# zhaoruiyang98/eftpipe

Hardware: AMD Instinct MI355X
Metric: theory P_l(k) evaluations/sec (single tracer, Nk=512, l=0,2,4) (higher is better)
Workload: dtype f64

## Files before the change

eftpipe_amd/csrc/eftb_kernels.hpp:

```cpp
#pragma once
#include <hip/hip_runtime.h>
#include <stdint.h>
#include <stdlib.h>

namespace eftb {

constexpr int NS = 80;
constexpr int NPOW = 257;
constexpr int NHALF = 128;
constexpr int NCH = 129;

constexpr int NROW = 24;

typedef double v4d __attribute__((ext_vector_type(4)));
typedef double v2d __attribute__((ext_vector_type(2)));

__device__ __forceinline__ void xcd_decode(int ntile, int& tile, int& group) {
    const int flat = blockIdx.x, ng = gridDim.x / ntile;
    if ((ng & 7) == 0) {
        const int slot = flat >> 3;
        tile = slot % ntile;
        group = (flat & 7) + 8 * (slot / ntile);
    } else {
        tile = flat % ntile;
        group = flat / ntile;
    }
}

template <bool LO>
__device__ __forceinline__ void prep_rows_body(int Nkin, int ntail, int nxtail, int KP1, int KP2, int KP3, int Bmax,
                                                        const double* __restrict__ Pin, const double* __restrict__ lnkin,
                                                        const double* __restrict__ lnxtail, const double* __restrict__ lnxxtail,
                                                        const double* __restrict__ wq2, double* __restrict__ A1, double* __restrict__ A2,
                                                        double* __restrict__ A2T, double* __restrict__ A3, int* __restrict__ status,
                                                        int ntail_lo, int nxtail_lo) {
    extern __shared__ double sm[];
    double* pin = sm;
    const int w = blockIdx.x, tid = threadIdx.x;
    bool bad = false;
    for (int j = tid; j < Nkin; j += blockDim.x) {
        const double v = Pin[(size_t)w * Nkin + j];
        pin[j] = v;
        bad = bad || !(fabs(v) <= 1.79769313486231570815e308) || (j >= Nkin - 2 && !(v > 0.0));
        if (LO) bad = bad || (j < 2 && !(v > 0.0));
    }
    if (bad && status) atomicMax(status, w + 1);
    __syncthreads();
    const double dln = lnkin[Nkin - 1] - lnkin[Nkin - 2];
    const double dlo = LO ? lnkin[1] - lnkin[0] : 0.0;
    if (A1) {
        const double slope = (log(pin[Nkin - 1]) - log(pin[Nkin - 2])) / dln;
        const double amp = pin[Nkin - 1] * exp(-slope * lnkin[Nkin - 1]);
        double slo = 0.0, alo = 0.0;
        if (LO && ntail_lo) {
            slo = (log(pin[1]) - log(pin[0])) / dlo;
            alo = pin[0] * exp(-slo * lnkin[0]);
        }
        const int nhi = ntail - (LO ? ntail_lo : 0);
        for (int j = tid; j < KP1; j += blockDim.x) A1[(size_t)w * KP1 + j] = j < Nkin ? pin[j] : 0.0;
        for (int j = tid; j < KP2; j += blockDim.x) {
            double v = j < Nkin ? pin[j] : (j < Nkin + ntail ? amp * exp(slope * lnxtail[j - Nkin]) : 0.0);
            if (LO && j >= Nkin + nhi && j < Nkin + ntail) v = alo * exp(slo * lnxtail[j - Nkin]);
            A2[(size_t)w * KP2 + j] = v;
            A2T[(size_t)j * Bmax + w] = v;
        }
    }
    if (A3) {
        const double q1 = pin[Nkin - 1] * wq2[1], q0 = pin[Nkin - 2] * wq2[0];
        const double slope = (log(q1) - log(q0)) / dln;
        const double amp = q1 * exp(-slope * lnkin[Nkin - 1]);
        double slo = 0.0, alo = 0.0;
        if (LO && nxtail_lo) {
            const double p0 = pin[0] * wq2[2], p1 = pin[1] * wq2[3];
            slo = (log(p1) - log(p0)) / dlo;
            alo = p0 * exp(-slo * lnkin[0]);
        }
        const int nhi = nxtail - (LO ? nxtail_lo : 0);
        for (int j = tid; j < KP3; j += blockDim.x) {
            double v = j < Nkin ? pin[j] : (j < Nkin + nxtail ? amp * exp(slope * lnxxtail[j - Nkin]) : 0.0);
            if (LO && j >= Nkin + nhi && j < Nkin + nxtail) v = alo * exp(slo * lnxxtail[j - Nkin]);
            A3[(size_t)w * KP3 + j] = v;
        }
    }
}

#define PREP_ROWS_PARAMS int Nkin, int ntail, int nxtail, int KP1, int KP2, int KP3, int Bmax, const double* __restrict__ Pin, \
    const double* __restrict__ lnkin, const double* __restrict__ lnxtail, const double* __restrict__ lnxxtail, const double* __restrict__ wq2, \
    double* __restrict__ A1, double* __restrict__ A2, double* __restrict__ A2T, double* __restrict__ A3, int* __restrict__ status
#define PREP_ROWS_ARGS Nkin, ntail, nxtail, KP1, KP2, KP3, Bmax, Pin, lnkin, lnxtail, lnxxtail, wq2, A1, A2, A2T, A3, status

__global__ __launch_bounds__(256) void prep_rows_kernel(PREP_ROWS_PARAMS) {
    prep_rows_body<false>(PREP_ROWS_ARGS, 0, 0);
}

__global__ __launch_bounds__(256) void prep_rows_lo_kernel(PREP_ROWS_PARAMS, int ntail_lo, int nxtail_lo) {
    prep_rows_body<true>(PREP_ROWS_ARGS, ntail_lo, nxtail_lo);
}

__device__ __forceinline__ void qf_body(int w, int nq, const double* __restrict__ fgrow, const double* __restrict__ Qpoly, double* __restrict__ Q) {
    const int tid = threadIdx.x;
    const double f = fgrow[w];
    for (int idx = tid; idx < 2 * nq; idx += blockDim.x) {
        const int a = idx / nq, rest = idx % nq;
        const double* c = Qpoly + ((size_t)(1 - a) * nq + rest) * 15;
        double cv[15];
#pragma unroll
        for (int p = 0; p < 15; ++p) cv[p] = c[p];
        const double f2 = f * f;
        double ev = cv[14], od = cv[13];
#pragma unroll
        for (int p = 12; p >= 0; p -= 2) {
            ev = fma(ev, f2, cv[p]);
            if (p >= 1) od = fma(od, f2, cv[p - 1]);
        }
        Q[(size_t)w * 2 * nq + idx] = fma(od, f, ev);
    }
}

__global__ __launch_bounds__(256) void prep_rows_qf_kernel(int B, PREP_ROWS_PARAMS, int nq, const double* __restrict__ fgrow,
                                                           const double* __restrict__ Qpoly, double* __restrict__ Q) {
    if ((int)blockIdx.x >= B) {
        qf_body(blockIdx.x - B, nq, fgrow, Qpoly, Q);
        return;
    }
    prep_rows_body<false>(PREP_ROWS_ARGS, 0, 0);
}

__global__ __launch_bounds__(256) void prep_rows_qf_lo_kernel(int B, PREP_ROWS_PARAMS, int nq, const double* __restrict__ fgrow,
                                                              const double* __restrict__ Qpoly, double* __restrict__ Q, int ntail_lo, int nxtail_lo) {
    if ((int)blockIdx.x >= B) {
        qf_body(blockIdx.x - B, nq, fgrow, Qpoly, Q);
        return;
    }
    prep_rows_body<true>(PREP_ROWS_ARGS, ntail_lo, nxtail_lo);
}
#undef PREP_ROWS_PARAMS
#undef PREP_ROWS_ARGS

constexpr int AD_T = NHALF + 2;
constexpr int AD_CH = 1;
constexpr int KSYN = 528;
constexpr int KLIN = 288;
constexpr int SYN_KPAD = 48;
constexpr int SYN_KC = 24;
static_assert(SYN_KPAD % SYN_KC == 0 && (32 * SYN_KC) % 256 == 0, "chunk must divide the padding and fill the staging threads");
constexpr int BAS22 = 8, BASC = 32;

__device__ __forceinline__ double readlane_f64(double v, int lane) {
    return __hiloint2double(__builtin_amdgcn_readlane(__double2hiint(v), lane), __builtin_amdgcn_readlane(__double2loint(v), lane));
}

template <int NC, int NW>
__global__ __launch_bounds__(64 * NW) void antidiag_kernel(int B, int Bmax, const double* __restrict__ coefT,
                                                           const double2* __restrict__ AD, double2* __restrict__ S) {
    constexpr int PB = 3, WPP = 2 * NC;
    static_assert(PB * WPP <= 64, "one wave-load must hold a block's weights");
    __shared__ double red[NW - 1][2 * NC][64];
    const int grp = blockIdx.y, jp = (grp & 1) ? NPOW - 1 - (int)blockIdx.x : (int)blockIdx.x;
    const int lane = threadIdx.x & 63, wave = threadIdx.x >> 6, w = grp * 64 + lane;
    const int wl = w < B ? w : B - 1;
    const int cnt = ((2 * NHALF + jp) >> 1) - jp + 1;
    const int per = (cnt + NW - 1) / NW, t0 = wave * per, t1 = min(cnt, t0 + per);
    const double* cr = coefT + wl;
    const double* ci = coefT + (size_t)NCH * Bmax + wl;
    double ar[NC], ai[NC];
#pragma unroll
    for (int q = 0; q < NC; ++q) ar[q] = ai[q] = 0.0;
    if (t0 < t1) {
        const double* adw = reinterpret_cast<const double*>(AD + ((size_t)jp * AD_T + t0) * NC);
        const int nw = (t1 - t0) * WPP;
        auto wload = [&](int blk) { return adw[min(blk * PB * WPP + lane, nw - 1)]; };
        double xr[PB], xi[PB], yr[PB], yi[PB];
        auto coef = [&](int t, int p) {
            const int n = jp + t, qn = n <= NHALF ? n : 2 * NHALF - n;
            xr[p] = cr[(size_t)qn * Bmax];
            xi[p] = ci[(size_t)qn * Bmax];
            yr[p] = cr[(size_t)t * Bmax];
            yi[p] = ci[(size_t)t * Bmax];
        };
        double wc = wload(0);
#pragma unroll
        for (int p = 0; p < PB; ++p) coef(min(t0 + p, t1 - 1), p);
        const int nblk = (t1 - t0 + PB - 1) / PB;
        for (int blk = 0; blk < nblk; ++blk) {
            const double wn = wload(blk + 1);
#pragma unroll
            for (int p = 0; p < PB; ++p) {
                const int t = t0 + blk * PB + p;
                const double on = t < t1 ? 1.0 : 0.0;
                const double xim = jp + t <= NHALF ? xi[p] : -xi[p], yim = -yi[p];
                const double pr = (xr[p] * yr[p] - xim * yim) * on, pi = (xr[p] * yim + xim * yr[p]) * on;
                __builtin_amdgcn_sched_barrier(0);
                coef(min(t + PB, t1 - 1), p);
                __builtin_amdgcn_sched_barrier(0);
#pragma unroll
                for (int q = 0; q < NC; ++q) {
                    const double mx = readlane_f64(wc, p * WPP + 2 * q), my = readlane_f64(wc, p * WPP + 2 * q + 1);
                    ar[q] = fma(mx, pr, fma(-my, pi, ar[q]));
                    ai[q] = fma(mx, pi, fma(my, pr, ai[q]));
                }
                __builtin_amdgcn_sched_barrier(0);
            }
            wc = wn;
        }
    }
    if (wave > 0) {
#pragma unroll
        for (int q = 0; q < NC; ++q) {
            red[wave - 1][2 * q][lane] = ar[q];
            red[wave - 1][2 * q + 1][lane] = ai[q];
        }
    }
    __syncthreads();
    if (wave == 0 && w < B) {
#pragma unroll
        for (int q = 0; q < NC; ++q) {
#pragma unroll
            for (int v = 0; v < NW - 1; ++v) {
                ar[q] += red[v][2 * q][lane];
                ai[q] += red[v][2 * q + 1][lane];
            }
            S[((size_t)w * NC + q) * NPOW + jp] = make_double2(ar[q], ai[q]);
        }
    }
}

template <int NC, int NW>
__global__ __launch_bounds__(64 * NW) void antidiag_nh_kernel(int B, int Bmax, const double* __restrict__ coefT,
                                                              const double2* __restrict__ AD, double2* __restrict__ S, int nh) {
    constexpr int PB = 3, WPP = 2 * NC;
    static_assert(PB * WPP <= 64, "one wave-load must hold a block's weights");
    __shared__ double red[NW - 1][2 * NC][64];
    const int npow = 2 * nh + 1, nch = nh + 1, adt = nh + 2;
    const int grp = blockIdx.y, jp = (grp & 1) ? npow - 1 - (int)blockIdx.x : (int)blockIdx.x;
    const int lane = threadIdx.x & 63, wave = threadIdx.x >> 6, w = grp * 64 + lane;
    const int wl = w < B ? w : B - 1;
    const int cnt = ((2 * nh + jp) >> 1) - jp + 1;
    const int per = (cnt + NW - 1) / NW, t0 = wave * per, t1 = min(cnt, t0 + per);
    const double* cr = coefT + wl;
    const double* ci = coefT + (size_t)nch * Bmax + wl;
    double ar[NC], ai[NC];
#pragma unroll
    for (int q = 0; q < NC; ++q) ar[q] = ai[q] = 0.0;
    if (t0 < t1) {
        const double* adw = reinterpret_cast<const double*>(AD + ((size_t)jp * adt + t0) * NC);
        const int nw = (t1 - t0) * WPP;
        auto wload = [&](int blk) { return adw[min(blk * PB * WPP + lane, nw - 1)]; };
        double xr[PB], xi[PB], yr[PB], yi[PB];
        auto coef = [&](int t, int p) {
            const int n = jp + t, qn = n <= nh ? n : 2 * nh - n;
            xr[p] = cr[(size_t)qn * Bmax];
            xi[p] = ci[(size_t)qn * Bmax];
            yr[p] = cr[(size_t)t * Bmax];
            yi[p] = ci[(size_t)t * Bmax];
        };
        double wc = wload(0);
#pragma unroll
        for (int p = 0; p < PB; ++p) coef(min(t0 + p, t1 - 1), p);
        const int nblk = (t1 - t0 + PB - 1) / PB;
        for (int blk = 0; blk < nblk; ++blk) {
            const double wn = wload(blk + 1);
#pragma unroll
            for (int p = 0; p < PB; ++p) {
                const int t = t0 + blk * PB + p;
                const double on = t < t1 ? 1.0 : 0.0;
                const double xim = jp + t <= nh ? xi[p] : -xi[p], yim = -yi[p];
                const double pr = (xr[p] * yr[p] - xim * yim) * on, pi = (xr[p] * yim + xim * yr[p]) * on;
                __builtin_amdgcn_sched_barrier(0);
                coef(min(t + PB, t1 - 1), p);
                __builtin_amdgcn_sched_barrier(0);
#pragma unroll
                for (int q = 0; q < NC; ++q) {
                    const double mx = readlane_f64(wc, p * WPP + 2 * q), my = readlane_f64(wc, p * WPP + 2 * q + 1);
                    ar[q] = fma(mx, pr, fma(-my, pi, ar[q]));
                    ai[q] = fma(mx, pi, fma(my, pr, ai[q]));
                }
                __builtin_amdgcn_sched_barrier(0);
            }
            wc = wn;
        }
    }
    if (wave > 0) {
#pragma unroll
        for (int q = 0; q < NC; ++q) {
            red[wave - 1][2 * q][lane] = ar[q];
            red[wave - 1][2 * q + 1][lane] = ai[q];
        }
    }
    __syncthreads();
    if (wave == 0 && w < B) {
#pragma unroll
        for (int q = 0; q < NC; ++q) {
#pragma unroll
            for (int v = 0; v < NW - 1; ++v) {
                ar[q] += red[v][2 * q][lane];
                ai[q] += red[v][2 * q + 1][lane];
            }
            S[((size_t)w * NC + q) * npow + jp] = make_double2(ar[q], ai[q]);
        }
    }
}

template <int NC>
__global__ __launch_bounds__(64) void build_rows_kernel(int sets, int Bmax, int Nl, int nlc, int nb, const double* __restrict__ coef,
                                                         const double2* __restrict__ S, const double2* __restrict__ mlj,
                                                         const double2* __restrict__ linvec, double* __restrict__ A22,
                                                         double* __restrict__ A13, double* __restrict__ ACF, double* __restrict__ ALC) {
    const int w = blockIdx.x, cf = blockIdx.y, jp = blockIdx.z * 64 + threadIdx.x;
    if (((sets >> cf) & 1) && jp < NPOW) {
        double zr[NC], zi[NC];
#pragma unroll
        for (int q = 0; q < NC; ++q) {
            zr[q] = zi[q] = 0.0;
#pragma unroll
            for (int ch = 0; ch < AD_CH; ++ch) {
                const double2 v = S[(((size_t)ch * Bmax + w) * NC + q) * NPOW + jp];
                zr[q] += v.x;
                zi[q] += v.y;
            }
        }
        const int o0 = jp == 0 ? 0 : 2 * jp - 1;
        if (cf == 0) {
#pragma unroll
            for (int q = 0; q < NC; ++q)
                if (q < nb) {
                    double* o = A22 + ((size_t)w * BAS22 + q) * KSYN;
                    o[o0] = zr[q];
                    if (jp) o[o0 + 1] = zi[q];
                }
        } else {
            for (int l = 0; l < Nl; ++l) {
                const double2 m = mlj[l * NPOW + jp];
#pragma unroll
                for (int q = 0; q < NC; ++q) {
                    double* o = ACF + ((size_t)w * BASC + l * NC + q) * KSYN;
                    o[o0] = m.x * zr[q] - m.y * zi[q];
                    if (jp) o[o0 + 1] = m.x * zi[q] + m.y * zr[q];
                }
            }
        }
    }
    if ((sets >> (2 + cf)) & 1) {
        const int nrows = cf == 0 ? 10 : nlc * Nl, v0 = cf == 0 ? 0 : 10;
        double* out = cf == 0 ? A13 + (size_t)w * 10 * KLIN : ALC + (size_t)w * nlc * Nl * KLIN;
        const double* c = coef + (size_t)w * 2 * NCH;
        for (int e = jp; e < nrows * NCH; e += 320) {
            const int row = e / NCH, mp = e % NCH, n = NHALF - mp;
            const double2 v = linvec[(size_t)(v0 + row) * NCH + n];
            const double cr = c[n], ci = n == NHALF ? 0.0 : c[NCH + n];
            double* o = out + (size_t)row * KLIN;
            if (mp == 0) o[0] = cr * v.x - ci * v.y;
            else {
                o[2 * mp - 1] = cr * v.x - ci * v.y;
                o[2 * mp] = cr * v.y + ci * v.x;
            }
        }
    }
}

__host__ __device__ constexpr int ksyn_of(int nh) { return (4 * nh + SYN_KPAD) / SYN_KPAD * SYN_KPAD; }
__host__ __device__ constexpr int klin_of(int nh) { return (2 * nh + SYN_KPAD) / SYN_KPAD * SYN_KPAD; }
static_assert(ksyn_of(NHALF) == KSYN && klin_of(NHALF) == KLIN, "row lengths of the default NFFT");

template <int NC>
__global__ __launch_bounds__(64) void build_rows_nh_kernel(int sets, int Bmax, int Nl, int nlc, int nb, const double* __restrict__ coef,
                                                            const double2* __restrict__ S, const double2* __restrict__ mlj,
                                                            const double2* __restrict__ linvec, double* __restrict__ A22,
                                                            double* __restrict__ A13, double* __restrict__ ACF, double* __restrict__ ALC, int nh) {
    const int npow = 2 * nh + 1, nch = nh + 1, ksyn = ksyn_of(nh), klin = klin_of(nh), zstride = 64 * (int)gridDim.z;
    const int w = blockIdx.x, cf = blockIdx.y, jp = blockIdx.z * 64 + threadIdx.x;
    if (((sets >> cf) & 1) && jp < npow) {
        double zr[NC], zi[NC];
#pragma unroll
        for (int q = 0; q < NC; ++q) {
            zr[q] = zi[q] = 0.0;
#pragma unroll
            for (int ch = 0; ch < AD_CH; ++ch) {
                const double2 v = S[(((size_t)ch * Bmax + w) * NC + q) * npow + jp];
                zr[q] += v.x;
                zi[q] += v.y;
            }
        }
        const int o0 = jp == 0 ? 0 : 2 * jp - 1;
        if (cf == 0) {
#pragma unroll
            for (int q = 0; q < NC; ++q)
                if (q < nb) {
                    double* o = A22 + ((size_t)w * BAS22 + q) * ksyn;
                    o[o0] = zr[q];
                    if (jp) o[o0 + 1] = zi[q];
                }
        } else {
            for (int l = 0; l < Nl; ++l) {
                const double2 m = mlj[l * npow + jp];
#pragma unroll
                for (int q = 0; q < NC; ++q) {
                    double* o = ACF + ((size_t)w * BASC + l * NC + q) * ksyn;
                    o[o0] = m.x * zr[q] - m.y * zi[q];
                    if (jp) o[o0 + 1] = m.x * zi[q] + m.y * zr[q];
                }
            }
        }
    }
    if ((sets >> (2 + cf)) & 1) {
        const int nrows = cf == 0 ? 10 : nlc * Nl, v0 = cf == 0 ? 0 : 10;
        double* out = cf == 0 ? A13 + (size_t)w * 10 * klin : ALC + (size_t)w * nlc * Nl * klin;
        const double* c = coef + (size_t)w * 2 * nch;
        for (int e = jp; e < nrows * nch; e += zstride) {
            const int row = e / nch, mp = e % nch, n = nh - mp;
            const double2 v = linvec[(size_t)(v0 + row) * nch + n];
            const double cr = c[n], ci = n == nh ? 0.0 : c[nch + n];
            double* o = out + (size_t)row * klin;
            if (mp == 0) o[0] = cr * v.x - ci * v.y;
            else {
                o[2 * mp - 1] = cr * v.x - ci * v.y;
                o[2 * mp] = cr * v.y + ci * v.x;
            }
        }
    }
}

__device__ inline double ipow(double f, int p) {
    double r = 1.0;
    for (int i = 0; i < p; ++i) r *= f;
    return r;
}

template <int NC>
__global__ __launch_bounds__(64) void build_rows_plk_kernel(int Bmax, int nb, const double* __restrict__ coef, const double2* __restrict__ S,
                                                             const double2* __restrict__ mlj, const double2* __restrict__ linvec,
                                                             const double* __restrict__ bias, const double* __restrict__ fgrow,
                                                             const double* __restrict__ l11, const double* __restrict__ lct,
                                                             const double* __restrict__ l22, const double* __restrict__ l13,
                                                             const int* __restrict__ grp, const double* __restrict__ exp22,
                                                             const double* __restrict__ expc, double* __restrict__ A22, double* __restrict__ A13,
                                                             double* __restrict__ ACF, double* __restrict__ ALC) {
    constexpr int NL = 3;
    __shared__ double s_cf[NL * 38];
    __shared__ double s_w[NL * NC];
    __shared__ double s_b[2 * NL];
    const int w = blockIdx.x, cf = blockIdx.y, jp = blockIdx.z * 64 + threadIdx.x;
    const double* bw = bias + (size_t)w * NROW;
    const double f = fgrow[w];
    for (int e = threadIdx.x; e < NL * 38; e += 64) {
        const int l = e / 38, bq = e % 38;
        s_cf[e] = bw[9 + grp[2 * bq]] * ipow(f, grp[2 * bq + 1]) * (bq < 28 ? l22[l * 28 + bq] : l13[l * 10 + (bq - 28)]);
    }
    if (threadIdx.x < 2 * NL) {
        const int a = threadIdx.x / NL, lp = threadIdx.x % NL;
        double v = 0.0;
        if (a == 0)
            for (int r = 0; r < 3; ++r) v = fma(bw[r], l11[lp * 3 + r], v);
        else
            for (int r = 0; r < 6; ++r) v = fma(bw[3 + r], lct[lp * 6 + r], v);
        s_b[threadIdx.x] = v;
    }
    __syncthreads();
    if (threadIdx.x < NL * NC) {
        const int l = threadIdx.x / NC, q = threadIdx.x % NC;
        double v0 = 0.0, v1 = 0.0;
        if (cf == 0) {
            if (q < nb)
                for (int b = 0; b < 28; b += 2) {
                    v0 = fma(s_cf[l * 38 + b], exp22[b * BAS22 + q], v0);
                    v1 = fma(s_cf[l * 38 + b + 1], exp22[(b + 1) * BAS22 + q], v1);
                }
        } else {
            for (int b = 0; b < 28; b += 2) {
                v0 = fma(s_cf[l * 38 + b], expc[(size_t)(l * 28 + b) * BASC + l * NC + q], v0);
                v1 = fma(s_cf[l * 38 + b + 1], expc[(size_t)(l * 28 + b + 1) * BASC + l * NC + q], v1);
            }
            for (int b = 0; b < 10; b += 2) {
                v0 = fma(s_cf[l * 38 + 28 + b], expc[(size_t)(NL * 28 + l * 10 + b) * BASC + l * NC + q], v0);
                v1 = fma(s_cf[l * 38 + 29 + b], expc[(size_t)(NL * 28 + l * 10 + b + 1) * BASC + l * NC + q], v1);
            }
        }
        s_w[threadIdx.x] = v0 + v1;
    }
    __syncthreads();
    if (jp < NPOW) {
        double zr[NC], zi[NC];
#pragma unroll
        for (int q = 0; q < NC; ++q) {
            zr[q] = zi[q] = 0.0;
#pragma unroll
            for (int ch = 0; ch < AD_CH; ++ch) {
                const double2 v = S[(((size_t)ch * Bmax + w) * NC + q) * NPOW + jp];
                zr[q] += v.x;
                zi[q] += v.y;
            }
        }
        const int o0 = jp == 0 ? 0 : 2 * jp - 1;
#pragma unroll
        for (int l = 0; l < NL; ++l) {
            double cr = 0.0, ci = 0.0;
#pragma unroll
            for (int q = 0; q < NC; ++q) {
                cr = fma(s_w[l * NC + q], zr[q], cr);
                ci = fma(s_w[l * NC + q], zi[q], ci);
            }
            if (cf == 0) {
                double* o = A22 + ((size_t)w * BAS22 + l) * KSYN;
                o[o0] = cr;
                if (jp) o[o0 + 1] = ci;
            } else {
                const double2 m = mlj[l * NPOW + jp];
                double* o = ACF + ((size_t)w * BASC + l) * KSYN;
                o[o0] = m.x * cr - m.y * ci;
                if (jp) o[o0 + 1] = m.x * ci + m.y * cr;
            }
        }
    }
    {
        const int nrows = cf == 0 ? NL : 2 * NL;
        double* out = cf == 0 ? A13 + (size_t)w * 10 * KLIN : ALC + (size_t)w * 2 * NL * KLIN;
        const double* c = coef + (size_t)w * 2 * NCH;
        for (int e = jp; e < nrows * NCH; e += 320) {
            const int row = e / NCH, mp = e % NCH, n = NHALF - mp;
            double vx, vy;
            if (cf == 0) {
                vx = vy = 0.0;
#pragma unroll
                for (int b = 0; b < 10; ++b) {
                    const double2 v = linvec[(size_t)b * NCH + n];
                    vx = fma(s_cf[row * 38 + 28 + b], v.x, vx);
                    vy = fma(s_cf[row * 38 + 28 + b], v.y, vy);
                }
            } else {
                const double2 v = linvec[(size_t)(10 + row) * NCH + n];
                vx = s_b[row] * v.x;
                vy = s_b[row] * v.y;
            }
            const double cr = c[n], ci = n == NHALF ? 0.0 : c[NCH + n];
            double* o = out + (size_t)row * KLIN;
            if (mp == 0) o[0] = cr * vx - ci * vy;
            else {
                o[2 * mp - 1] = cr * vx - ci * vy;
                o[2 * mp] = cr * vy + ci * vx;
            }
        }
    }
}

template <int NC>
__global__ __launch_bounds__(64) void build_rows_plk_nh_kernel(int Bmax, int nb, const double* __restrict__ coef, const double2* __restrict__ S,
                                                    const double2* __restrict__ mlj, const double2* __restrict__ linvec,
                                                    const double* __restrict__ bias, const double* __restrict__ fgrow,
                                                    const double* __restrict__ l11, const double* __restrict__ lct,
                                                    const double* __restrict__ l22, const double* __restrict__ l13,
                                                    const int* __restrict__ grp, const double* __restrict__ exp22,
                                                    const double* __restrict__ expc, double* __restrict__ A22, double* __restrict__ A13,
                                                    double* __restrict__ ACF, double* __restrict__ ALC, int nh) {
    constexpr int NL = 3;
    const int npow = 2 * nh + 1, nch = nh + 1, ksyn = ksyn_of(nh), klin = klin_of(nh), zstride = 64 * (int)gridDim.z;
    __shared__ double s_cf[NL * 38];
    __shared__ double s_w[NL * NC];
    __shared__ double s_b[2 * NL];
    const int w = blockIdx.x, cf = blockIdx.y, jp = blockIdx.z * 64 + threadIdx.x;
    const double* bw = bias + (size_t)w * NROW;
    const double f = fgrow[w];
    for (int e = threadIdx.x; e < NL * 38; e += 64) {
        const int l = e / 38, bq = e % 38;
        s_cf[e] = bw[9 + grp[2 * bq]] * ipow(f, grp[2 * bq + 1]) * (bq < 28 ? l22[l * 28 + bq] : l13[l * 10 + (bq - 28)]);
    }
    if (threadIdx.x < 2 * NL) {
        const int a = threadIdx.x / NL, lp = threadIdx.x % NL;
        double v = 0.0;
        if (a == 0)
            for (int r = 0; r < 3; ++r) v = fma(bw[r], l11[lp * 3 + r], v);
        else
            for (int r = 0; r < 6; ++r) v = fma(bw[3 + r], lct[lp * 6 + r], v);
        s_b[threadIdx.x] = v;
    }
    __syncthreads();
    if (threadIdx.x < NL * NC) {
        const int l = threadIdx.x / NC, q = threadIdx.x % NC;
        double v0 = 0.0, v1 = 0.0;
        if (cf == 0) {
            if (q < nb)
                for (int b = 0; b < 28; b += 2) {
                    v0 = fma(s_cf[l * 38 + b], exp22[b * BAS22 + q], v0);
                    v1 = fma(s_cf[l * 38 + b + 1], exp22[(b + 1) * BAS22 + q], v1);
                }
        } else {
            for (int b = 0; b < 28; b += 2) {
                v0 = fma(s_cf[l * 38 + b], expc[(size_t)(l * 28 + b) * BASC + l * NC + q], v0);
                v1 = fma(s_cf[l * 38 + b + 1], expc[(size_t)(l * 28 + b + 1) * BASC + l * NC + q], v1);
            }
            for (int b = 0; b < 10; b += 2) {
                v0 = fma(s_cf[l * 38 + 28 + b], expc[(size_t)(NL * 28 + l * 10 + b) * BASC + l * NC + q], v0);
                v1 = fma(s_cf[l * 38 + 29 + b], expc[(size_t)(NL * 28 + l * 10 + b + 1) * BASC + l * NC + q], v1);
            }
        }
        s_w[threadIdx.x] = v0 + v1;
    }
    __syncthreads();
    if (jp < npow) {
        double zr[NC], zi[NC];
#pragma unroll
        for (int q = 0; q < NC; ++q) {
            zr[q] = zi[q] = 0.0;
#pragma unroll
            for (int ch = 0; ch < AD_CH; ++ch) {
// ... 3925 lines not shown
```

Baseline: 1.837 million.

## Broadcast antidiagonal weights via DPP row_newbcast FMAs instead of readlane

Rewrites the antidiagonal complex-accumulation kernel so per-term weights are held in 16-lane-replicated registers and applied with v_fmac_f64_dpp row_newbcast inline asm, replacing the pair of scalar readlanes per weight. Coefficient loads now use a 4-deep ring with a block of 8 terms, and the weight registers are refilled as each one is consumed. The two near-duplicate kernels are merged into one shared body. The goal is to remove the readlane/SGPR round trips and the masking multiply from the inner loop. In exchange the code relies on hand-written DPP asm, which is gfx-specific and more fragile.

```diff
diff --git a/eftpipe_amd/csrc/eftb_kernels.hpp b/eftpipe_amd/csrc/eftb_kernels.hpp
--- a/eftpipe_amd/csrc/eftb_kernels.hpp
+++ b/eftpipe_amd/csrc/eftb_kernels.hpp
@@ -2,6 +2,7 @@
 #include <hip/hip_runtime.h>
 #include <stdint.h>
 #include <stdlib.h>
+#include <type_traits>
 
 namespace eftb {
 
@@ -150,90 +151,29 @@
     return __hiloint2double(__builtin_amdgcn_readlane(__double2hiint(v), lane), __builtin_amdgcn_readlane(__double2loint(v), lane));
 }
 
+template <int N, bool NEG>
+__device__ __forceinline__ void bcast_fmac(double& acc, double tab, double b) {
+    static_assert(N >= 0 && N < 16, "row_newbcast takes a lane of the row");
+    if constexpr (NEG) asm("v_fmac_f64_dpp %0, -%1, %2 row_newbcast:%3 row_mask:0xf bank_mask:0xf" : "+v"(acc) : "v"(tab), "v"(b), "n"(N));
+    else asm("v_fmac_f64_dpp %0, %1, %2 row_newbcast:%3 row_mask:0xf bank_mask:0xf" : "+v"(acc) : "v"(tab), "v"(b), "n"(N));
+}
+template <int I0, int I1, typename F>
+__device__ __forceinline__ void static_for(F&& f) {
+    if constexpr (I0 < I1) {
+        f(std::integral_constant<int, I0>{});
+        static_for<I0 + 1, I1>(f);
+    }
+}
+
 template <int NC, int NW>
-__global__ __launch_bounds__(64 * NW) void antidiag_kernel(int B, int Bmax, const double* __restrict__ coefT,
-                                                           const double2* __restrict__ AD, double2* __restrict__ S) {
-    constexpr int PB = 3, WPP = 2 * NC;
-    static_assert(PB * WPP <= 64, "one wave-load must hold a block's weights");
-    __shared__ double red[NW - 1][2 * NC][64];
-    const int grp = blockIdx.y, jp = (grp & 1) ? NPOW - 1 - (int)blockIdx.x : (int)blockIdx.x;
-    const int lane = threadIdx.x & 63, wave = threadIdx.x >> 6, w = grp * 64 + lane;
-    const int wl = w < B ? w : B - 1;
-    const int cnt = ((2 * NHALF + jp) >> 1) - jp + 1;
-    const int per = (cnt + NW - 1) / NW, t0 = wave * per, t1 = min(cnt, t0 + per);
-    const double* cr = coefT + wl;
-    const double* ci = coefT + (size_t)NCH * Bmax + wl;
-    double ar[NC], ai[NC];
-#pragma unroll
-    for (int q = 0; q < NC; ++q) ar[q] = ai[q] = 0.0;
-    if (t0 < t1) {
-        const double* adw = reinterpret_cast<const double*>(AD + ((size_t)jp * AD_T + t0) * NC);
-        const int nw = (t1 - t0) * WPP;
-        auto wload = [&](int blk) { return adw[min(blk * PB * WPP + lane, nw - 1)]; };
-        double xr[PB], xi[PB], yr[PB], yi[PB];
-        auto coef = [&](int t, int p) {
-            const int n = jp + t, qn = n <= NHALF ? n : 2 * NHALF - n;
-            xr[p] = cr[(size_t)qn * Bmax];
-            xi[p] = ci[(size_t)qn * Bmax];
-            yr[p] = cr[(size_t)t * Bmax];
-            yi[p] = ci[(size_t)t * Bmax];
-        };
-        double wc = wload(0);
-#pragma unroll
-        for (int p = 0; p < PB; ++p) coef(min(t0 + p, t1 - 1), p);
-        const int nblk = (t1 - t0 + PB - 1) / PB;
-        for (int blk = 0; blk < nblk; ++blk) {
-            const double wn = wload(blk + 1);
-#pragma unroll
-            for (int p = 0; p < PB; ++p) {
-                const int t = t0 + blk * PB + p;
-                const double on = t < t1 ? 1.0 : 0.0;
-                const double xim = jp + t <= NHALF ? xi[p] : -xi[p], yim = -yi[p];
-                const double pr = (xr[p] * yr[p] - xim * yim) * on, pi = (xr[p] * yim + xim * yr[p]) * on;
-                __builtin_amdgcn_sched_barrier(0);
-                coef(min(t + PB, t1 - 1), p);
-                __builtin_amdgcn_sched_barrier(0);
-#pragma unroll
-                for (int q = 0; q < NC; ++q) {
-                    const double mx = readlane_f64(wc, p * WPP + 2 * q), my = readlane_f64(wc, p * WPP + 2 * q + 1);
-                    ar[q] = fma(mx, pr, fma(-my, pi, ar[q]));
-                    ai[q] = fma(mx, pi, fma(my, pr, ai[q]));
-                }
-                __builtin_amdgcn_sched_barrier(0);
-            }
-            wc = wn;
-        }
-    }
-    if (wave > 0) {
-#pragma unroll
-        for (int q = 0; q < NC; ++q) {
-            red[wave - 1][2 * q][lane] = ar[q];
-            red[wave - 1][2 * q + 1][lane] = ai[q];
-        }
-    }
-    __syncthreads();
-    if (wave == 0 && w < B) {
-#pragma unroll
-        for (int q = 0; q < NC; ++q) {
-#pragma unroll
-            for (int v = 0; v < NW - 1; ++v) {
-                ar[q] += red[v][2 * q][lane];
-                ai[q] += red[v][2 * q + 1][lane];
-            }
-            S[((size_t)w * NC + q) * NPOW + jp] = make_double2(ar[q], ai[q]);
-        }
-    }
-}
-
-template <int NC, int NW>
-__global__ __launch_bounds__(64 * NW) void antidiag_nh_kernel(int B, int Bmax, const double* __restrict__ coefT,
-                                                              const double2* __restrict__ AD, double2* __restrict__ S, int nh) {
-    constexpr int PB = 3, WPP = 2 * NC;
-    static_assert(PB * WPP <= 64, "one wave-load must hold a block's weights");
+__device__ __forceinline__ void antidiag_body(int B, int Bmax, const double* __restrict__ coefT, const double2* __restrict__ AD,
+                                              double2* __restrict__ S, const int nh) {
+    constexpr int PB = 8, WPP = 2 * NC, RING = 4;
+    static_assert(PB * WPP == 16 * NC && PB % RING == 0, "a block's weights fill NC registers of 16; the ring's slots repeat from block to block");
     __shared__ double red[NW - 1][2 * NC][64];
     const int npow = 2 * nh + 1, nch = nh + 1, adt = nh + 2;
     const int grp = blockIdx.y, jp = (grp & 1) ? npow - 1 - (int)blockIdx.x : (int)blockIdx.x;
-    const int lane = threadIdx.x & 63, wave = threadIdx.x >> 6, w = grp * 64 + lane;
+    const int lane = threadIdx.x & 63, wave = __builtin_amdgcn_readfirstlane(threadIdx.x >> 6), w = grp * 64 + lane;
     const int wl = w < B ? w : B - 1;
     const int cnt = ((2 * nh + jp) >> 1) - jp + 1;
     const int per = (cnt + NW - 1) / NW, t0 = wave * per, t1 = min(cnt, t0 + per);
@@ -243,10 +183,10 @@
 #pragma unroll
     for (int q = 0; q < NC; ++q) ar[q] = ai[q] = 0.0;
     if (t0 < t1) {
-        const double* adw = reinterpret_cast<const double*>(AD + ((size_t)jp * adt + t0) * NC);
-        const int nw = (t1 - t0) * WPP;
-        auto wload = [&](int blk) { return adw[min(blk * PB * WPP + lane, nw - 1)]; };
-        double xr[PB], xi[PB], yr[PB], yi[PB];
+        const double* adw = reinterpret_cast<const double*>(AD + ((size_t)jp * adt + t0) * NC) + (lane & 15);
+        const int wlast = (t1 - t0) * WPP - 1 - (lane & 15);
+        double W[NC];
+        double xr[RING], xi[RING], yr[RING], yi[RING];
         auto coef = [&](int t, int p) {
             const int n = jp + t, qn = n <= nh ? n : 2 * nh - n;
             xr[p] = cr[(size_t)qn * Bmax];
@@ -254,30 +194,41 @@
             yr[p] = cr[(size_t)t * Bmax];
             yi[p] = ci[(size_t)t * Bmax];
         };
-        double wc = wload(0);
-#pragma unroll
-        for (int p = 0; p < PB; ++p) coef(min(t0 + p, t1 - 1), p);
-        const int nblk = (t1 - t0 + PB - 1) / PB;
-        for (int blk = 0; blk < nblk; ++blk) {
-            const double wn = wload(blk + 1);
-#pragma unroll
-            for (int p = 0; p < PB; ++p) {
-                const int t = t0 + blk * PB + p;
-                const double on = t < t1 ? 1.0 : 0.0;
-                const double xim = jp + t <= nh ? xi[p] : -xi[p], yim = -yi[p];
-                const double pr = (xr[p] * yr[p] - xim * yim) * on, pi = (xr[p] * yim + xim * yr[p]) * on;
+#pragma unroll
+        for (int m = 0; m < NC; ++m) W[m] = adw[min(16 * m, wlast)];
+#pragma unroll
+        for (int p = 0; p < RING; ++p) {
+            __builtin_amdgcn_sched_barrier(0);
+            coef(min(t0 + p, t1 - 1), p);
+        }
+        for (int tb = t0, wb = PB * WPP; tb < t1; tb += PB, wb += PB * WPP) {
+            static_for<0, PB>([&](auto pc) {
+                constexpr int p = pc, r = p % RING;
+                const int t = tb + p;
+                const double xim = jp + t <= nh ? xi[r] : -xi[r];
+                double pr = fma(xim, yi[r], xr[r] * yr[r]), pi = fma(xim, yr[r], -(yi[r] * xr[r]));
+                asm volatile("" : "+v"(pr), "+v"(pi));
                 __builtin_amdgcn_sched_barrier(0);
-                coef(min(t + PB, t1 - 1), p);
+                coef(min(t + RING, t1 - 1), r);
                 __builtin_amdgcn_sched_barrier(0);
-#pragma unroll
-                for (int q = 0; q < NC; ++q) {
-                    const double mx = readlane_f64(wc, p * WPP + 2 * q), my = readlane_f64(wc, p * WPP + 2 * q + 1);
-                    ar[q] = fma(mx, pr, fma(-my, pi, ar[q]));
-                    ai[q] = fma(mx, pi, fma(my, pr, ai[q]));
+                if (t < t1) {
+                    static_for<0, NC>([&](auto qc) {
+                        constexpr int q = qc, f = p * WPP + 2 * q;
+                        bcast_fmac<(f + 1) % 16, true>(ar[q], W[f / 16], pi);
+                        bcast_fmac<(f + 1) % 16, false>(ai[q], W[f / 16], pr);
+                    });
+                    static_for<0, NC>([&](auto qc) {
+                        constexpr int q = qc, f = p * WPP + 2 * q;
+                        bcast_fmac<f % 16, false>(ar[q], W[f / 16], pr);
+                        bcast_fmac<f % 16, false>(ai[q], W[f / 16], pi);
+                    });
                 }
                 __builtin_amdgcn_sched_barrier(0);
-            }
-            wc = wn;
+                static_for<0, NC>([&](auto mc) {
+                    constexpr int m = mc;
+                    if constexpr ((16 * m + 15) / WPP == p) W[m] = adw[min(wb + 16 * m, wlast)];
+                });
+            });
         }
     }
     if (wave > 0) {
@@ -299,6 +250,16 @@
             S[((size_t)w * NC + q) * npow + jp] = make_double2(ar[q], ai[q]);
         }
     }
+}
+template <int NC, int NW>
+__global__ __launch_bounds__(64 * NW) void antidiag_kernel(int B, int Bmax, const double* __restrict__ coefT,
+                                                           const double2* __restrict__ AD, double2* __restrict__ S) {
+    antidiag_body<NC, NW>(B, Bmax, coefT, AD, S, NHALF);
+}
+template <int NC, int NW>
+__global__ __launch_bounds__(64 * NW) void antidiag_nh_kernel(int B, int Bmax, const double* __restrict__ coefT,
+                                                              const double2* __restrict__ AD, double2* __restrict__ S, int nh) {
+    antidiag_body<NC, NW>(B, Bmax, coefT, AD, S, nh);
 }
 
 template <int NC>
```

Measured after the change: 1.705 million. 0.928x the previous value.

## Restructure antidiag kernel with LDS weight broadcast and split conjugate segments

Applied to the files above, without the earlier changes.

Reworks the antidiagonal accumulation kernel so weights are staged through a double-buffered per-wave LDS slot and read as double2 vectors, replacing per-element readlane broadcasts. The loop is split into non-conjugate and conjugate segments at compile time to remove per-iteration branching and the masking multiply. Coefficient loads use a scalar row base plus a single vector byte offset to cut address arithmetic. It also sets a waves-per-EU occupancy hint. The changes add LDS traffic and register-pressure constraints in exchange for fewer cross-lane ops and less VALU address math.

```diff
diff --git a/eftpipe_amd/csrc/eftb_kernels.hpp b/eftpipe_amd/csrc/eftb_kernels.hpp
--- a/eftpipe_amd/csrc/eftb_kernels.hpp
+++ b/eftpipe_amd/csrc/eftb_kernels.hpp
@@ -151,58 +151,95 @@
 }
 
 template <int NC, int NW>
-__global__ __launch_bounds__(64 * NW) void antidiag_kernel(int B, int Bmax, const double* __restrict__ coefT,
+__global__ __launch_bounds__(64 * NW) __attribute__((amdgpu_waves_per_eu(5))) void antidiag_kernel(int B, int Bmax, const double* __restrict__ coefT,
                                                            const double2* __restrict__ AD, double2* __restrict__ S) {
     constexpr int PB = 3, WPP = 2 * NC;
     static_assert(PB * WPP <= 64, "one wave-load must hold a block's weights");
     __shared__ double red[NW - 1][2 * NC][64];
+    __shared__ __attribute__((aligned(16))) double wts[NW][2][64];
     const int grp = blockIdx.y, jp = (grp & 1) ? NPOW - 1 - (int)blockIdx.x : (int)blockIdx.x;
-    const int lane = threadIdx.x & 63, wave = threadIdx.x >> 6, w = grp * 64 + lane;
-    const int wl = w < B ? w : B - 1;
+    const int lane = threadIdx.x & 63, wave = __builtin_amdgcn_readfirstlane(threadIdx.x >> 6);
+    const int w = grp * 64 + lane;
+    const unsigned wo8 = 8u * (unsigned)(w < B ? w : B - 1);
     const int cnt = ((2 * NHALF + jp) >> 1) - jp + 1;
     const int per = (cnt + NW - 1) / NW, t0 = wave * per, t1 = min(cnt, t0 + per);
-    const double* cr = coefT + wl;
-    const double* ci = coefT + (size_t)NCH * Bmax + wl;
     double ar[NC], ai[NC];
 #pragma unroll
     for (int q = 0; q < NC; ++q) ar[q] = ai[q] = 0.0;
     if (t0 < t1) {
         const double* adw = reinterpret_cast<const double*>(AD + ((size_t)jp * AD_T + t0) * NC);
         const int nw = (t1 - t0) * WPP;
-        auto wload = [&](int blk) { return adw[min(blk * PB * WPP + lane, nw - 1)]; };
-        double xr[PB], xi[PB], yr[PB], yi[PB];
-        auto coef = [&](int t, int p) {
-            const int n = jp + t, qn = n <= NHALF ? n : 2 * NHALF - n;
-            xr[p] = cr[(size_t)qn * Bmax];
-            xi[p] = ci[(size_t)qn * Bmax];
-            yr[p] = cr[(size_t)t * Bmax];
-            yi[p] = ci[(size_t)t * Bmax];
+        double* wslot = &wts[wave][0][0];
+        auto segment = [&](auto conj, int tb, int te) {
+            constexpr bool CONJ = decltype(conj)::value;
+            if (tb >= te) return;
+            const int wo = (tb - t0) * WPP;
+            auto wload = [&](int blk) { return adw[min(wo + blk * PB * WPP + lane, nw - 1)]; };
+            double xr[PB], xi[PB], yr[PB], yi[PB];
+            auto coef = [&](int t, int p) {
+                const int n = jp + t, qn = CONJ ? 2 * NHALF - n : n;
+                const char* rxr = reinterpret_cast<const char*>(coefT + (size_t)qn * Bmax);
+                const char* rxi = reinterpret_cast<const char*>(coefT + (size_t)(NCH + qn) * Bmax);
+                const char* ryr = reinterpret_cast<const char*>(coefT + (size_t)t * Bmax);
+                const char* ryi = reinterpret_cast<const char*>(coefT + (size_t)(NCH + t) * Bmax);
+                unsigned o = wo8;
+                asm volatile("" : "+v"(o));
+                xr[p] = *reinterpret_cast<const double*>(rxr + o);
+                xi[p] = *reinterpret_cast<const double*>(rxi + o);
+                yr[p] = *reinterpret_cast<const double*>(ryr + o);
+                yi[p] = *reinterpret_cast<const double*>(ryi + o);
+            };
+            auto pair = [&](int t, int p, const double* wb, bool reload) {
+                const double2* wq = reinterpret_cast<const double2*>(wb) + p * NC;
+                constexpr int QB = 2, NQB = (NC + QB - 1) / QB;
+                double2 m[NQB][QB];
+#pragma unroll
+                for (int q = 0; q < QB; ++q) m[0][q] = wq[q];
+                const double xim = CONJ ? -xi[p] : xi[p];
+                double pr = __builtin_fma(xim, yi[p], xr[p] * yr[p]), pi = __builtin_fma(xim, yr[p], -(xr[p] * yi[p]));
+                asm volatile("" : "+v"(pr), "+v"(pi));
+                __builtin_amdgcn_sched_barrier(0);
+                if (reload) coef(min(t + PB, te - 1), p);
+                __builtin_amdgcn_sched_barrier(0);
+#pragma unroll
+                for (int b = 0; b < NQB; ++b) {
+#pragma unroll
+                    for (int q = 0; q < QB; ++q)
+                        if (b + 1 < NQB && (b + 1) * QB + q < NC) m[b + 1][q] = wq[(b + 1) * QB + q];
+                    __builtin_amdgcn_sched_barrier(0);
+#pragma unroll
+                    for (int q = 0; q < QB; ++q)
+                        if (b * QB + q < NC) {
+                            const double mx = m[b][q].x, my = m[b][q].y;
+                            ar[b * QB + q] = __builtin_fma(mx, pr, __builtin_fma(-my, pi, ar[b * QB + q]));
+                            ai[b * QB + q] = __builtin_fma(mx, pi, __builtin_fma(my, pr, ai[b * QB + q]));
+                        }
+                    __builtin_amdgcn_sched_barrier(0);
+                }
+            };
+            const int nfull = (te - tb) / PB, ntail = (te - tb) - nfull * PB;
+            double wn = wload(0);
+#pragma unroll
+            for (int p = 0; p < PB; ++p) coef(min(tb + p, te - 1), p);
+            wslot[lane] = wn;
+            for (int blk = 0; blk < nfull; ++blk) {
+                wn = wload(blk + 1);
+                const double* wb = wslot + (blk & 1) * 64;
+                __builtin_amdgcn_fence(__ATOMIC_ACQUIRE, "wavefront");
+#pragma unroll
+                for (int p = 0; p < PB; ++p) pair(tb + blk * PB + p, p, wb, true);
+                wslot[((blk + 1) & 1) * 64 + lane] = wn;
+                __builtin_amdgcn_fence(__ATOMIC_RELEASE, "wavefront");
+            }
+            const double* wb = wslot + (nfull & 1) * 64;
+            __builtin_amdgcn_fence(__ATOMIC_ACQUIRE, "wavefront");
+#pragma unroll
+            for (int p = 0; p < PB - 1; ++p)
+                if (p < ntail) pair(tb + nfull * PB + p, p, wb, false);
         };
-        double wc = wload(0);
-#pragma unroll
-        for (int p = 0; p < PB; ++p) coef(min(t0 + p, t1 - 1), p);
-        const int nblk = (t1 - t0 + PB - 1) / PB;
-        for (int blk = 0; blk < nblk; ++blk) {
-            const double wn = wload(blk + 1);
-#pragma unroll
-            for (int p = 0; p < PB; ++p) {
-                const int t = t0 + blk * PB + p;
-                const double on = t < t1 ? 1.0 : 0.0;
-                const double xim = jp + t <= NHALF ? xi[p] : -xi[p], yim = -yi[p];
-                const double pr = (xr[p] * yr[p] - xim * yim) * on, pi = (xr[p] * yim + xim * yr[p]) * on;
-                __builtin_amdgcn_sched_barrier(0);
-                coef(min(t + PB, t1 - 1), p);
-                __builtin_amdgcn_sched_barrier(0);
-#pragma unroll
-                for (int q = 0; q < NC; ++q) {
-                    const double mx = readlane_f64(wc, p * WPP + 2 * q), my = readlane_f64(wc, p * WPP + 2 * q + 1);
-                    ar[q] = fma(mx, pr, fma(-my, pi, ar[q]));
-                    ai[q] = fma(mx, pi, fma(my, pr, ai[q]));
-                }
-                __builtin_amdgcn_sched_barrier(0);
-            }
-            wc = wn;
-        }
+        const int ts = max(t0, min(t1, NHALF - jp + 1));
+        segment(std::false_type{}, t0, ts);
+        segment(std::true_type{}, ts, t1);
     }
     if (wave > 0) {
 #pragma unroll
```

Result: no change. 1.856 million before, 1.837 million after, median of 2 (-1.0%).
